# mryab/learning-at-home

Measured on NVIDIA H100. Metric: DMoE training samples/sec (whole job, device-timed, max over ranks), higher is better.
Workload: dtype bf16

## Files before the change

### learning-at-home_b200/csrc/moe.cu

```cuda
#include <cfloat>

#include "sm90.cuh"

namespace lah {

constexpr int MAX_WORLD = 8;
constexpr int MAX_GRID_DIMS = 4;
constexpr int MAX_K = 8;
constexpr long long SPIN_TIMEOUT_CYCLES = 20000000000ll;

struct Peers {
    char* base[MAX_WORLD];
    int world;
    int me;
    unsigned long long* wait_ns;
    int* step_ctr;
    int spin_timeout_ms;
    char* mc_base;
};

__device__ __forceinline__ void multimem_st_release_u32(void* mc_addr, int v) {
    asm volatile("multimem.st.release.sys.global.u32 [%0], %1;" ::"l"(mc_addr), "r"(v) : "memory");
}
__device__ __forceinline__ void multimem_st_u32(void* mc_addr, int v) {
// ... 611 lines not shown
}

__global__ void alive_from_heartbeats_kernel(const long long* hb, unsigned char* alive, int E, long long now_ms, long long max_age_ms) {
    const int e = blockIdx.x * blockDim.x + threadIdx.x;
    if (e < E) alive[e] = (hb[e] > 0 && now_ms - hb[e] <= max_age_ms) ? 1 : 0;
}

__global__ void step_begin_kernel(int* step_ctr, int epoch_delta, long long token_delta) {
    step_ctr[0] += epoch_delta;
    *reinterpret_cast<long long*>(step_ctr + 2) += token_delta;
}

struct CombineArgs {
    long long src_off;
    const int* idx;
    const int* pair_row;
    const float* w;
    bf16* out;
    int B, k, H, E_loc;
    long long flags_off;
    int slot, epoch, do_signal, do_wait;
    int* status;
    const int* route_owner;
};

template <int VEC_PER_LANE, bool ADD>
__global__ void __launch_bounds__(256) combine_rows_kernel(Peers peers, CombineArgs a, const bf16* __restrict__ addend) {
    const int warp = threadIdx.x >> 5, lane = threadIdx.x & 31;
    if (a.do_signal || a.do_wait) a.epoch = epoch_of(peers, a.epoch);
    if (a.do_signal && blockIdx.x == 0 && threadIdx.x < 32) {
        signal_all_ranks(peers, a.flags_off, a.slot, a.epoch, threadIdx.x);
    }
    if (a.do_wait) {
        if (threadIdx.x < peers.world) {
            const int* f = reinterpret_cast<const int*>(peers.base[peers.me] + a.flags_off) + a.slot * MAX_WORLD + threadIdx.x;
            const unsigned long long t0 = globaltimer_ns();
            spin_until_ge(f, a.epoch, a.status, peers.spin_timeout_ms, threadIdx.x);
            if (blockIdx.x == 0) account_wait(peers, t0, peers.world);
        }
        __syncthreads();
    }
    const int b = blockIdx.x * 8 + warp;
    if (b >= a.B) return;
    float acc[VEC_PER_LANE * 8];
    if constexpr (ADD) {
        const int4* ap = reinterpret_cast<const int4*>(addend + static_cast<long long>(b) * a.H);
#pragma unroll
        for (int v = 0; v < VEC_PER_LANE; ++v) {
            const int4 q = __ldg(ap + v * 32 + lane);
            const uint32_t u[4] = {(uint32_t)q.x, (uint32_t)q.y, (uint32_t)q.z, (uint32_t)q.w};
#pragma unroll
            for (int t = 0; t < 4; ++t) {
// ... 517 lines not shown
    if (!g_peers_set) return -10;
    ScatterArgs a;
    a.src = (const bf16*)src; a.scale = scale; a.idx = idx; a.pos = pos; a.dst_row = dst_row; a.pair_row = pair_row;
    a.dst_off = dst_off; a.flags_off = flags_off; a.slot = slot; a.epoch = epoch; a.num_pairs = num_pairs; a.k = k;
    a.H = H; a.E_loc = E_loc; a.max_rows = max_rows; a.group_off = group_off; a.group_rows = group_rows;
    a.pair_blocks = (num_pairs + 7) / 8; a.align = align; a.done_counter = done_counter; a.status = status;
    a.route_owner = route_owner; a.num_groups = num_groups > 0 ? num_groups : E_loc;
    const int pad_blocks = a.num_groups < 64 ? a.num_groups : 64;
    const int grid = a.pair_blocks + pad_blocks;
    if (H == 256) scatter_rows_kernel<1><<<grid, 256, 0, st>>>(g_peers, a);
    else if (H == 512) scatter_rows_kernel<2><<<grid, 256, 0, st>>>(g_peers, a);
    else if (H == 1024) scatter_rows_kernel<4><<<grid, 256, 0, st>>>(g_peers, a);
    else return -2;
    return -(int)cudaGetLastError();
}

int lah_signal_wait(long long flags_off, int slot, int epoch, int do_signal, int do_wait, int* status,
                    cudaStream_t st) {
    if (!g_peers_set) return -10;
    signal_wait_kernel<<<1, 32, 0, st>>>(g_peers, flags_off, slot, epoch, do_signal, do_wait, status);
    return -(int)cudaGetLastError();
}

int lah_combine_rows(long long src_off, const int* idx, const int* pair_row, const float* w, void* out, int B, int k,
                     int H, int E_loc, long long flags_off, int slot, int epoch, int do_signal, int do_wait, int* status,
                     const int* route_owner, const void* addend, cudaStream_t st) {
    if (!g_peers_set) return -10;
    if (B <= 0) return 0;
    CombineArgs a;
    a.src_off = src_off; a.idx = idx; a.pair_row = pair_row; a.w = w; a.out = (bf16*)out; a.B = B; a.k = k; a.H = H;
    a.E_loc = E_loc; a.flags_off = flags_off; a.slot = slot; a.epoch = epoch; a.do_signal = do_signal; a.do_wait = do_wait;
    a.status = status; a.route_owner = route_owner;
    const int grid = (B + 7) / 8;
    const bf16* add = (const bf16*)addend;
    if (add && (reinterpret_cast<uintptr_t>(add) % 16)) return -3;
#define LAH_COMBINE(V)                                                                   \
    if (add) combine_rows_kernel<V, true><<<grid, 256, 0, st>>>(g_peers, a, add);        \
    else combine_rows_kernel<V, false><<<grid, 256, 0, st>>>(g_peers, a, nullptr);
    if (H == 256) { LAH_COMBINE(1) }
    else if (H == 512) { LAH_COMBINE(2) }
    else if (H == 1024) { LAH_COMBINE(4) }
    else return -2;
#undef LAH_COMBINE
    return -(int)cudaGetLastError();
}

int lah_gate_bwd(long long yo_off, const void* grad, const int* idx, const int* pair_row, const float* w,
                 float* dlogits, int B, int k, int H, int E_loc, const int* grid_sizes, int ndim, const int* route_owner,
                 cudaStream_t st) {
    if (!g_peers_set) return -10;
    if (B <= 0) return 0;
    GridSpec gs;
// ... 104 lines not shown
```

### learning-at-home_b200/csrc/small_m.cu

```cuda
#include "sm90.cuh"
#include <climits>

namespace lah {
namespace smallm {

constexpr int BM = 128;
constexpr int BK = 64;
constexpr int MMA_K = 16;
constexpr int BN_MAX = 128;
constexpr int NUM_THREADS = 288;

namespace sab {

constexpr int STAGES = 6;
constexpr int A_BYTES = BM * BK * 2;
constexpr int B_BYTES = BN_MAX * BK * 2;
constexpr int STAGE_BYTES = A_BYTES + B_BYTES;
constexpr int BAR_OFFSET = STAGES * STAGE_BYTES;
constexpr int QD = 4;
constexpr int MAX_G = 1023;
constexpr int CUM_OFFSET = BAR_OFFSET + (2 * STAGES + 2 * QD) * 8 + QD * 4 + 16;
constexpr int SMEM_TOTAL = CUM_OFFSET + (MAX_G + 1) * 4 + 1024;
static_assert(SMEM_TOTAL <= 232448, "shared memory budget");

struct Params {
    int G, M_out, K;
    const int* group_off;
// ... 136 lines not shown
    const int num_kb = p.K / BK;

    if (warp == 8) {
        if (lane != 0) return;
        if (p.wait_flags) {
            const int epoch = p.wait_epoch + (p.epoch_base ? *p.epoch_base : 0);
            const unsigned long long t_wait = globaltimer_ns();
            for (int sidx = 0; sidx < p.wait_count; ++sidx)
                spin_flag_ft(p.wait_flags + sidx, epoch, p.status, sidx, p.epoch_base ? p.epoch_base[1] : 0);
            if (blockIdx.x == 0) atomicAdd(reinterpret_cast<unsigned long long*>(p.status + 2), globaltimer_ns() - t_wait);
            fence_proxy_async_global();
        }
        int stage = 0, qi = 0;
        uint32_t phase = 0, qphase = 0;
        while (true) {
            const int tile = atomicAdd(p.tile_counter, 1);
            mbar_wait(&q_empty[qi], qphase ^ 1);
            q_tile[qi] = tile;
            mbar_arrive(&q_full[qi]);
            if (++qi == QD) {
                qi = 0;
                qphase ^= 1;
            }
            if (tile >= total) break;
            const int gc = tile / m_slices, ms = tile - gc * m_slices;
            const int g = find_group(cum, p.G, gc);
            const int n0 = (gc - cum[g]) * BN_MAX;
            const int rows = __ldg(p.group_rows + g);
            const int off = __ldg(p.group_off + g);
            const int box = box_rows_of(min(rows - n0, BN_MAX));
            const CUtensorMap* tmB = box == 16 ? &tmB16 : (box == 32 ? &tmB32 : (box == 64 ? &tmB64 : &tmB128));
            for (int kb = 0; kb < num_kb; ++kb) {
                mbar_wait(&empty_bar[stage], phase ^ 1);
                uint8_t* sa = smem + stage * STAGE_BYTES;
                uint8_t* sb = sa + A_BYTES;
                const int k = kb * BK;
                mbar_arrive_expect_tx(&full_bar[stage], A_BYTES + box * 128);
                if (!A_MN) {
                    tma_load_3d(sa, &tmA, &full_bar[stage], k, ms * BM, g);
                } else {
#pragma unroll
                    for (int i = 0; i < BM / 64; ++i)
                        tma_load_3d(sa + i * (BK * 128), &tmA, &full_bar[stage], ms * BM + i * 64, k, g);
                }
                tma_load_2d(sb, tmB, &full_bar[stage], k, off + n0);
                if (++stage == STAGES) {
                    stage = 0;
// ... 53 lines not shown
static_assert(ST_STAGES <= CHUNKS, "the producer issues a tile's first ST_STAGES chunks before its remaining k-blocks");
static_assert(OP_STAGE_BYTES % 1024 == 0 && SUB_BYTES % 1024 == 0, "128-B swizzle atoms need 1 KB alignment");
static_assert(SMEM_TOTAL <= 232448, "shared memory budget");

struct Params {
    int G, N, K;
    const int* group_off;
    const int* group_rows;
    const int* skip;
    const int* step;
    float* p;
    float* m;
    float* v;
    float* vmax;
    bf16* p_bf16;
    float lr, beta1, beta2, eps;
    int amsgrad;
    float wd;
    int* tile_counter;
    const int* poison;
};
static_assert(sizeof(Params) == 128 && sizeof(Params) % alignof(CUtensorMap) == 0, "Params layout");

constexpr int WD_NONE = 0, WD_L2 = 1, WD_DECOUPLED = 2;

struct Tile {
    int g, mt, nt;
};

template <bool SPLIT>
struct StateMaps {
    CUtensorMap a[SPLIT ? 5 : 4];
};
constexpr int PLANE_COLS = 64;
constexpr int PLANE_BYTES = ARR_BYTES / 2;
static_assert(PLANE_BYTES == (BN_MAX / PLANE_COLS) * SUB_BYTES, "a plane box has the rows and bytes of an fp32 box");

template <bool SPLIT>
__device__ __forceinline__ void state_chunk_tma(const StateMaps<SPLIT>& tm, int n_arr, uint8_t* ss, uint64_t* bar, int col0,
                                                int srow, int c) {
    if constexpr (SPLIT) {
        for (int a = 0; a < 2; ++a)
#pragma unroll
            for (int q = 0; q < BN_MAX / PLANE_COLS; ++q) {
                uint8_t* s = ss + a * PLANE_BYTES + q * SUB_BYTES;
                if (bar) tma_load_3d(s, &tm.a[a], bar, col0 + q * PLANE_COLS, BAND_ROWS * c, srow / 16);
                else tma_store_3d(&tm.a[a], s, col0 + q * PLANE_COLS, BAND_ROWS * c, srow / 16);
            }
    }
    for (int a = SPLIT ? 1 : 0; a < n_arr; ++a)
#pragma unroll
        for (int q = 0; q < BN_MAX / SUB_COLS; ++q) {
            uint8_t* s = ss + a * ARR_BYTES + q * SUB_BYTES;
            const CUtensorMap* m = &tm.a[SPLIT ? a + 1 : a];
            if (bar) tma_load_3d(s, m, bar, col0 + q * SUB_COLS, BAND_ROWS * c, srow / 16);
            else tma_store_3d(m, s, col0 + q * SUB_COLS, BAND_ROWS * c, srow / 16);
        }
}

template <int WD, bool DEV_LR, bool SPLIT>
__global__ void __launch_bounds__(NUM_THREADS, 1)
wgrad_adam_kernel(const Params p, const __grid_constant__ CUtensorMap tmDY, const __grid_constant__ CUtensorMap tmX,
                  const __grid_constant__ StateMaps<SPLIT> tmS, const float* __restrict__ lr_dev) {
    extern __shared__ uint8_t smem_raw[];
    uint8_t* smem = reinterpret_cast<uint8_t*>((reinterpret_cast<uintptr_t>(smem_raw) + 1023) & ~uintptr_t(1023));
    uint8_t* st_smem = smem + ST_OFFSET;
    uint64_t* op_full = reinterpret_cast<uint64_t*>(smem + BAR_OFFSET);
    uint64_t* op_empty = op_full + OP_STAGES;
    uint64_t* st_full = op_empty + OP_STAGES;
    uint64_t* st_empty = st_full + ST_STAGES;
    uint64_t* q_full = st_empty + ST_STAGES;
    uint64_t* q_empty = q_full + QD;
    volatile int* q_tile = reinterpret_cast<volatile int*>(q_empty + QD);

    const int warp = threadIdx.x >> 5;
    const int lane = threadIdx.x & 31;
    if (p.poison && (*p.poison & 1)) return;
    const int n_arr = p.amsgrad ? 4 : 3;

    if (warp == 8 && lane == 0) {
        tma_prefetch_desc(&tmDY);
        tma_prefetch_desc(&tmX);
        for (int a = 0; a < n_arr + (SPLIT ? 1 : 0); ++a) tma_prefetch_desc(&tmS.a[a]);
        for (int i = 0; i < OP_STAGES; ++i) {
            mbar_init(&op_full[i], 1);
            mbar_init(&op_empty[i], 8);
        }
        for (int i = 0; i < ST_STAGES; ++i) {
            mbar_init(&st_full[i], 1);
            mbar_init(&st_empty[i], 1);
        }
        for (int i = 0; i < QD; ++i) {
            mbar_init(&q_full[i], 1);
            mbar_init(&q_empty[i], 8);
        }
        fence_mbar_init();
    }
    __syncthreads();

    const int n_tiles = p.K / BN_MAX;
    const int tiles_per_group = (p.N / BM) * n_tiles;
    const int total = p.G * tiles_per_group;
    auto decode = [&](int tile) {
        Tile t;
        t.g = tile / tiles_per_group;
        const int r = tile - t.g * tiles_per_group;
        t.mt = r / n_tiles;
        t.nt = r - t.mt * n_tiles;
        return t;
    };

    if (warp == 8) {
        if (lane != 0) return;
        uint32_t phase = 0, qphase = 0, sphase = 0;
        int qi = 0, stage = 0, sstage = 0;
        while (true) {
            int tile;
            while (true) {
                tile = atomicAdd(p.tile_counter, 1);
                if (tile >= total) break;
                const int g = tile / tiles_per_group;
                if (__ldg(p.group_rows + g) > 0 && !(p.skip && __ldg(p.skip + 2 * g) >= 0)) break;
                atomicMax(p.tile_counter, (g + 1) * tiles_per_group);
            }
            mbar_wait(&q_empty[qi], qphase ^ 1);
            q_tile[qi] = tile;
            mbar_arrive(&q_full[qi]);
            if (++qi == QD) {
                qi = 0;
                qphase ^= 1;
            }
            if (tile >= total) break;
            const Tile t = decode(tile);
            const int off = __ldg(p.group_off + t.g), rows = __ldg(p.group_rows + t.g);
            const int srow = t.g * p.N + t.mt * BM;
            auto load_chunk = [&](int c) {
                mbar_wait(&st_empty[sstage], sphase ^ 1);
                mbar_arrive_expect_tx(&st_full[sstage], n_arr * ARR_BYTES);
                state_chunk_tma(tmS, n_arr, st_smem + sstage * ST_STAGE_BYTES, &st_full[sstage], t.nt * BN_MAX, srow, c);
                if (++sstage == ST_STAGES) {
                    sstage = 0;
                    sphase ^= 1;
                }
// ... 164 lines not shown
                    acc[4 * j] = acc[4 * j + 2];
                    acc[4 * j + 1] = acc[4 * j + 3];
                }
            }
        }
    }
    if (threadIdx.x == 0) tma_store_wait<0>();
}

}
}
}

using namespace lah;
using namespace lah::smallm;

extern "C" const int* lah_get_epoch_base();

static int* tile_counter() {
    static int* ctr = nullptr;
    if (!ctr) {
        if (cudaMalloc(&ctr, 256) != cudaSuccess) return nullptr;
        cudaMemset(ctr, 0, 256);
    }
    return ctr;
}
static const int* g_poison = nullptr;

extern "C" {

int lah_set_poison_word(const int* status) {
    g_poison = status;
    return 0;
}
const int* lah_get_poison_word() { return g_poison; }

int lah_swapab_linear(const void* x, long long ldx, int x_rows, const void* W, int G, int M_out, int K, int a_mn,
                      void* out, long long ldo, const int* group_off, const int* group_rows, const float* bias,
                      const void* residual, long long ldr, const int* wait_flags, int wait_count, int wait_epoch,
                      int* status, int max_ctas, cudaStream_t st) {
    if ((K % BK) || (M_out % BM) || (ldx % 8) || G > sab::MAX_G) return -2;
    CUtensorMap tmA, tmB[4];
    if (!a_mn) {
        uint64_t dims[3] = {(uint64_t)K, (uint64_t)M_out, (uint64_t)G};
        uint64_t str[2] = {(uint64_t)K * 2, (uint64_t)M_out * K * 2};
        uint32_t box[3] = {BK, BM, 1};
        int r = make_tmap(&tmA, CU_TENSOR_MAP_DATA_TYPE_BFLOAT16, 3, W, dims, str, box);
        if (r) return r;
    } else {
        uint64_t dims[3] = {(uint64_t)M_out, (uint64_t)K, (uint64_t)G};
        uint64_t str[2] = {(uint64_t)M_out * 2, (uint64_t)M_out * K * 2};
        uint32_t box[3] = {64, BK, 1};
        int r = make_tmap(&tmA, CU_TENSOR_MAP_DATA_TYPE_BFLOAT16, 3, W, dims, str, box);
        if (r) return r;
    }
    const uint32_t boxes[4] = {16, 32, 64, 128};
    for (int i = 0; i < 4; ++i) {
        uint64_t dims[2] = {(uint64_t)K, (uint64_t)x_rows};
        uint64_t str[1] = {(uint64_t)ldx * 2};
        uint32_t box[2] = {BK, boxes[i]};
        int r = make_tmap(&tmB[i], CU_TENSOR_MAP_DATA_TYPE_BFLOAT16, 2, x, dims, str, box);
        if (r) return r;
    }
    sab::Params p;
    p.G = G; p.M_out = M_out; p.K = K; p.group_off = group_off; p.group_rows = group_rows; p.out = (bf16*)out; p.ldo = ldo;
    p.bias = bias; p.residual = (const bf16*)residual; p.ldr = ldr; p.wait_flags = wait_flags; p.wait_count = wait_count;
    p.wait_epoch = wait_epoch; p.epoch_base = lah_get_epoch_base(); p.status = status;
    p.tile_counter = tile_counter();
    if (!p.tile_counter) return -3;
    const long long total = 1ll * (M_out / BM) * (G + x_rows / BN_MAX);
    if (total <= 0 || G <= 0) return 0;
    if (cudaMemsetAsync(p.tile_counter, 0, sizeof(int), st) != cudaSuccess) return -4;
    const int ctas = persistent_grid(total, max_ctas);
    if (!a_mn) {
        if (int e = set_max_dynamic_smem<sab::swapab_kernel<false>>(sab::SMEM_TOTAL)) return e;
        sab::swapab_kernel<false><<<ctas, NUM_THREADS, sab::SMEM_TOTAL, st>>>(p, tmA, tmB[0], tmB[1], tmB[2], tmB[3]);
    } else {
        if (int e = set_max_dynamic_smem<sab::swapab_kernel<true>>(sab::SMEM_TOTAL)) return e;
        sab::swapab_kernel<true><<<ctas, NUM_THREADS, sab::SMEM_TOTAL, st>>>(p, tmA, tmB[0], tmB[1], tmB[2], tmB[3]);
    }
    return -(int)cudaGetLastError();
}

}

template <int WD, bool DEV_LR, bool SPLIT>
static int launch_wgrad_adam(const wa::Params& a, const CUtensorMap& tmDY, const CUtensorMap& tmX,
                             const wa::StateMaps<SPLIT>& tmS, const float* lr_dev, int ctas, cudaStream_t st) {
    if (int e = set_max_dynamic_smem<wa::wgrad_adam_kernel<WD, DEV_LR, SPLIT>>(wa::SMEM_TOTAL)) return e;
    wa::wgrad_adam_kernel<WD, DEV_LR, SPLIT><<<ctas, NUM_THREADS, wa::SMEM_TOTAL, st>>>(a, tmDY, tmX, tmS, lr_dev);
    return -(int)cudaGetLastError();
}

template <bool SPLIT>
static int wgrad_adam(const void* dy, long long lddy, const void* x, long long ldx, int total_rows, int G, int N, int K,
                      const int* group_off, const int* group_rows, const int* skip, const int* step, void* p, void* lo,
                      float* m, float* v, float* vmax, void* p_bf16, float lr, const float* lr_dev, float beta1, float beta2,
                      float eps, int amsgrad, float weight_decay, float decay, int decoupled, int max_ctas, cudaStream_t st) {
    if ((N % BM) || (K % BN_MAX) || (lddy % 8) || (ldx % 8) || 1ll * G * N > INT_MAX) return -2;
    if (decoupled && weight_decay != 0.f) return -2;
    if (amsgrad && !vmax) return -2;
    CUtensorMap tmDY, tmX;
    wa::StateMaps<SPLIT> tmS;
    {
        void* arrs[5] = {p, m, v, amsgrad ? vmax : (float*)m, nullptr};
        if (SPLIT) {
            arrs[1] = lo; arrs[2] = m; arrs[3] = v; arrs[4] = amsgrad ? vmax : m;
        }
        uint64_t dims[3] = {(uint64_t)K, 16, (uint64_t)G * N / 16};
        uint64_t str[2] = {(uint64_t)K * 4, (uint64_t)K * 64};
        uint32_t box[3] = {wa::SUB_COLS, wa::BAND_ROWS, BM / 16};
        for (int a = 0; a < (SPLIT ? 5 : 4); ++a) {
            int r;
            if (SPLIT && a < 2) {
                uint64_t pstr[2] = {(uint64_t)K * 2, (uint64_t)K * 32};
                uint32_t pbox[3] = {wa::PLANE_COLS, wa::BAND_ROWS, BM / 16};
                r = make_tmap(&tmS.a[a], CU_TENSOR_MAP_DATA_TYPE_BFLOAT16, 3, arrs[a], dims, pstr, pbox);
            } else {
                r = make_tmap(&tmS.a[a], CU_TENSOR_MAP_DATA_TYPE_FLOAT32, 3, arrs[a], dims, str, box);
            }
            if (r) return r;
// ... 2 lines not shown
    {
        uint64_t dims[2] = {(uint64_t)N, (uint64_t)total_rows};
        uint64_t str[1] = {(uint64_t)lddy * 2};
        uint32_t box[2] = {64, wa::WBK};
        int r = make_tmap(&tmDY, CU_TENSOR_MAP_DATA_TYPE_BFLOAT16, 2, dy, dims, str, box);
        if (r) return r;
    }
    {
        uint64_t dims[2] = {(uint64_t)K, (uint64_t)total_rows};
        uint64_t str[1] = {(uint64_t)ldx * 2};
        uint32_t box[2] = {64, wa::WBK};
        int r = make_tmap(&tmX, CU_TENSOR_MAP_DATA_TYPE_BFLOAT16, 2, x, dims, str, box);
        if (r) return r;
    }
    wa::Params a;
    a.G = G; a.N = N; a.K = K; a.group_off = group_off; a.group_rows = group_rows; a.skip = skip; a.step = step;
    a.p = SPLIT ? nullptr : (float*)p; a.m = m; a.v = v; a.vmax = vmax; a.p_bf16 = (bf16*)p_bf16; a.lr = lr; a.beta1 = beta1; a.beta2 = beta2; a.eps = eps; a.amsgrad = amsgrad;
    a.wd = decoupled ? decay : weight_decay;
    a.tile_counter = tile_counter() ? tile_counter() + 16 : nullptr;
    a.poison = g_poison;
    if (!a.tile_counter) return -3;
    const long long total = 1ll * G * (N / BM) * (K / BN_MAX);
    if (total <= 0) return 0;
    if (cudaMemsetAsync(a.tile_counter, 0, sizeof(int), st) != cudaSuccess) return -4;
    const int ctas = persistent_grid(total, max_ctas);
    if (lr_dev) {
        if (decoupled) return launch_wgrad_adam<wa::WD_DECOUPLED, true, SPLIT>(a, tmDY, tmX, tmS, lr_dev, ctas, st);
        if (weight_decay != 0.f) return launch_wgrad_adam<wa::WD_L2, true, SPLIT>(a, tmDY, tmX, tmS, lr_dev, ctas, st);
        return launch_wgrad_adam<wa::WD_NONE, true, SPLIT>(a, tmDY, tmX, tmS, lr_dev, ctas, st);
    }
    if (decoupled) return launch_wgrad_adam<wa::WD_DECOUPLED, false, SPLIT>(a, tmDY, tmX, tmS, nullptr, ctas, st);
    if (weight_decay != 0.f) return launch_wgrad_adam<wa::WD_L2, false, SPLIT>(a, tmDY, tmX, tmS, nullptr, ctas, st);
    return launch_wgrad_adam<wa::WD_NONE, false, SPLIT>(a, tmDY, tmX, tmS, nullptr, ctas, st);
}

extern "C" {

int lah_wgrad_adam(const void* dy, long long lddy, const void* x, long long ldx, int total_rows, int G, int N, int K,
                   const int* group_off, const int* group_rows, const int* skip, const int* step, float* p, float* m,
                   float* v, float* vmax, void* p_bf16, float lr, const float* lr_dev, float beta1, float beta2, float eps,
                   int amsgrad, float weight_decay, float decay, int decoupled, int max_ctas, cudaStream_t st) {
    return wgrad_adam<false>(dy, lddy, x, ldx, total_rows, G, N, K, group_off, group_rows, skip, step, p, nullptr, m, v,
                             vmax, p_bf16, lr, lr_dev, beta1, beta2, eps, amsgrad, weight_decay, decay, decoupled, max_ctas,
                             st);
}

int lah_wgrad_adam_split(const void* dy, long long lddy, const void* x, long long ldx, int total_rows, int G, int N, int K,
                         const int* group_off, const int* group_rows, const int* skip, const int* step, void* hi, void* lo,
                         float* m, float* v, float* vmax, float lr, const float* lr_dev, float beta1, float beta2, float eps,
                         int amsgrad, float weight_decay, float decay, int decoupled, int max_ctas, cudaStream_t st) {
    if (!hi || !lo) return -2;
    return wgrad_adam<true>(dy, lddy, x, ldx, total_rows, G, N, K, group_off, group_rows, skip, step, hi, lo, m, v, vmax,
                            nullptr, lr, lr_dev, beta1, beta2, eps, amsgrad, weight_decay, decay, decoupled, max_ctas, st);
}

}
```

### learning-at-home_b200/ops/kernels.py

```python
import ctypes
import math

import torch
import torch.nn.functional as F

from . import native
from .native import c_void_p, c_int, c_ll, c_float, ptr, stream_ptr

c_ull = ctypes.c_ulonglong
_configured = False

SLOT_COUNTS, SLOT_DISPATCH, SLOT_OUTPUT, SLOT_GRAD, SLOT_DINPUT, SLOT_TRAINER, SLOT_BARRIER, SLOT_SHADOW = range(8)
NUM_SLOTS = 8
MAX_WORLD = 8
STATUS_TIMEOUT, STATUS_OVERFLOW = 1, 2


def _lib():
    global _configured
    lib = native.cuda_lib()
    if _configured:
        return lib
    P, I, L, Fl = c_void_p, c_int, c_ll, c_float
    sigs = {
        "lah_ln_relu_fwd": [P, P, P, P, P, P, P, I, I, I, I, P],
        "lah_ln_relu_bwd": [P, P, P, P, P, P, P, P, P, P, P, P, I, I, I, I, P, P],
        "lah_grouped_colsum": [P, L, P, P, I, P, I, I, P],
        "lah_set_step_counters": [P],
        "lah_set_multicast": [c_ull],
        "lah_set_poison_word": [P],
        "lah_nvls_allreduce": [L, L, Fl, P],
        "lah_heartbeat": [L, I, I, L, P],
        "lah_alive_from_heartbeats": [P, P, I, L, L, P],
        "lah_set_spin_timeout_ms": [I],
        "lah_step_begin": [I, L, P],
        "lah_swapab_linear": [P, L, I, P, I, I, I, I, P, L, P, P, P, P, L, P, I, I, P, I, P],
        "lah_wgrad_adam": [P, L, P, L, I, I, I, I, P, P, P, P, P, P, P, P, P, Fl, P, Fl, Fl, Fl, I, Fl, Fl, I, I, P],
        "lah_wgrad_adam_split": [P, L, P, L, I, I, I, I, P, P, P, P, P, P, P, P, P, Fl, P, Fl, Fl, Fl, I, Fl, Fl, I, I, P],
        "lah_ln_relu_fwd_q": [P, P, P, P, P, P, P, I, I, I, P, P, P],
        "lah_set_peers": [P, I, I],
        "lah_set_wait_counter": [P],
        "lah_gate_topk": [P, I, P, I, I, P, Fl, c_ull, L, P, P, P, P, P, P],
        "lah_expert_bias_update": [P, I, I, P, Fl, P, P],
        "lah_layout_exchange": [L, L, I, I, I, I, I, I, I, P, P, P, P, P, P, P, I, Fl, I, P, P, P, P, P],
        "lah_scatter_rows": [P, P, P, P, P, P, L, L, I, I, I, I, I, I, I, I, P, P, P, P, P, I, P],
        "lah_pull_shadow": [P, I, I, L, L, I, P, I, P],
        "lah_zero_slots": [P, I, P, I, I, I, I, P],
        "lah_signal_wait": [L, I, I, I, I, P, P],
        "lah_combine_rows": [L, P, P, P, P, I, I, I, I, L, I, I, I, I, P, P, P, P],
        "lah_gate_bwd": [L, P, P, P, P, P, I, I, I, I, P, I, P, P],
        "lah_router_loss_fwd": [P, I, P, I, P, P, I, P, P, P, P, P, P, P],
        "lah_router_loss_bwd": [P, I, P, I, P, P, P, P, Fl, Fl, P, P],
        "lah_adam_step": [P, P, P, P, P, P, I, P, I, P, P, I, Fl, P, Fl, Fl, Fl, Fl, I, I, I, L, P, Fl, I, P, L, I, I, I, Fl,
                          I, P],
        "lah_bump_steps": [P, P, I, P],
        "lah_cast_bf16": [P, P, L, P],
        "lah_split_master": [P, P, P, P, L, I, P],
        "lah_attention_fwd": [P, P, P, L, I, I, I, c_ull, I, Fl, P, P],
        "lah_attention_bwd": [P, P, P, P, P, P, P, L, I, I, I, c_ull, I, Fl, P, P],
        "lah_attention_fwd_causal": [P, P, P, L, I, I, I, c_ull, I, Fl, P],
        "lah_attention_bwd_causal": [P, P, P, P, P, P, P, L, I, I, I, c_ull, I, Fl, P],
        "lah_pack_key_mask": [P, P, L, I, P],
        "lah_dropout_mask": [P, I, I, I, I, I, c_ull, I, P],
        "lah_dropout_ew": [I, P, P, P, L, I, c_ull, I, I, Fl, P],
        "lah_rms_norm_fwd": [P, P, P, P, I, I, Fl, P, I, P],
        "lah_rms_norm_bwd": [P, P, P, P, P, P, P, I, I, I, P, P, P],
        "lah_swiglu_fwd": [P, P, L, I, P],
        "lah_swiglu_bwd": [P, P, P, L, I, P],
        "lah_symm_alloc": [c_ull, ctypes.POINTER(c_void_p)],
        "lah_symm_free": [P],
        "lah_symm_get_handle": [P, ctypes.c_char_p],
        "lah_symm_open_handle": [ctypes.c_char_p, ctypes.POINTER(c_void_p)],
# ... 277 lines not shown
    native.count_launch()


def scatter_rows(src, scale, idx, pos, dst_row, pair_row, dst_off, flags_off, slot, epoch, k, E_loc, max_rows,
                 group_off, group_rows, done_counter, status, align=128, route_owner=None, num_groups=0):
    num_pairs = idx.numel()
    H = src.shape[1]
    assert src.is_contiguous() and src.dtype == torch.bfloat16
    native.check(_lib().lah_scatter_rows(ptr(src), ptr(scale), ptr(idx), ptr(pos), ptr(dst_row), ptr(pair_row), dst_off,
                                         flags_off, slot, epoch, num_pairs, k, H, E_loc, max_rows, align, ptr(group_off),
                                         ptr(group_rows), ptr(done_counter), ptr(status), ptr(route_owner),
                                         int(num_groups), stream_ptr()),
                 "lah_scatter_rows")
    native.count_launch()


def signal_wait(flags_off, slot, epoch, status, *, signal=True, wait=True):
    native.check(_lib().lah_signal_wait(flags_off, slot, epoch, int(signal), int(wait), ptr(status), stream_ptr()),
                 "lah_signal_wait")
    native.count_launch()


def combine_rows(src_off, idx, pair_row, w, out, k, E_loc, *, flags_off=0, slot=0, epoch=0, signal=False, wait=False,
                 status=None, route_owner=None, addend=None):
    B, H = out.shape
    if addend is not None:
        _bf16_rows(addend, "combine_rows addend", (B, H))
        if addend.data_ptr() % 16:
            raise ValueError("combine_rows: the addend must be 16-byte aligned")
    native.check(_lib().lah_combine_rows(src_off, ptr(idx), ptr(pair_row), ptr(w), ptr(out), B, k, H, E_loc, flags_off,
                                         slot, epoch, int(signal), int(wait), ptr(status), ptr(route_owner),
                                         ptr(addend), stream_ptr()),
                 "lah_combine_rows")
    native.count_launch()
    return out


def combine_rows_ref(src, idx, pair_row, w=None, addend=None):
    present = ((idx >= 0) & (pair_row >= 0)).double()
    if w is not None:
        present = present * w.double()
    terms = src.double()[pair_row.clamp(min=0).long()] * present.unsqueeze(-1)
    total = terms.sum(1)
    if addend is not None:
        total = total + addend.double()
    return total.to(torch.bfloat16)


def gate_bwd(yo_off, grad, idx, pair_row, w, dlogits, k, E_loc, grid_size, route_owner=None):
    B, H = grad.shape
    assert grad.is_contiguous() and grad.dtype == torch.bfloat16 and dlogits.dtype == torch.float32
    native.check(_lib().lah_gate_bwd(yo_off, ptr(grad), ptr(idx), ptr(pair_row), ptr(w), ptr(dlogits), B, k, H, E_loc,
                                     ctypes.cast(_grid_array(grid_size), c_void_p), len(grid_size), ptr(route_owner),
                                     stream_ptr()),
                 "lah_gate_bwd")
# ... 391 lines not shown
                                          wait_epoch, ptr(wait_status), int(max_ctas), stream_ptr()),
                 "lah_swapab_linear")
    native.count_launch()
    return out


def swapab_linear_ref(x, w, group_off, group_rows, *, bias=None, residual=None, w_is_kn=False):
    off, rows = group_off.tolist(), group_rows.tolist()
    M_out = w.shape[2] if w_is_kn else w.shape[1]
    out = torch.zeros(x.shape[0], M_out, dtype=torch.float32, device=x.device)
    for g, (o, r) in enumerate(zip(off, rows)):
        if r <= 0:
            continue
        wg = w[g].float()
        y = x[o:o + r].float() @ (wg if w_is_kn else wg.t())
        if bias is not None:
            y = y + bias.view(w.shape[0], M_out)[g]
        if residual is not None:
            y = y + residual[o:o + r].float()
        out[o:o + r] = y
    return out


def wgrad_adam(dy, x, group_off, group_rows, *, p, m, v, vmax, p_bf16, step, skip=None, lr=1e-3, betas=(0.9, 0.999),
               eps=1e-8, amsgrad=True, weight_decay=0.0, decoupled=False, max_ctas=0, lr_dev=None, p_lo=None):
    G, N, Kd = (p if p_lo is None else p_lo).shape
    assert dy.shape[1] == N and x.shape[1] == Kd and dy.shape[0] == x.shape[0]
    assert dy.dtype == torch.bfloat16 and x.dtype == torch.bfloat16
    if p_lo is None:
        assert p.is_contiguous() and p.dtype == torch.float32
    else:
        assert p is None and p_lo.dtype == torch.int16 and p_bf16.dtype == torch.bfloat16
        assert p_lo.is_contiguous() and p_bf16.is_contiguous() and p_bf16.shape[1:] == p_lo.shape[1:]
    if amsgrad and vmax is None:
        raise ValueError("wgrad_adam: amsgrad needs a vmax tensor (vmax=None only with amsgrad=False)")
    if lr_dev is not None:
        _check_lr_dev(lr_dev)
    l2, decay = weight_decay_args(lr, weight_decay, decoupled)
    common = (ptr(dy), dy.stride(0), ptr(x), x.stride(0), dy.shape[0], G, N, Kd, ptr(group_off), ptr(group_rows),
              ptr(skip), ptr(step))
    tail = (lr, ptr(lr_dev), betas[0], betas[1], eps, int(amsgrad), l2, decay, int(bool(decoupled and weight_decay)),
            int(max_ctas), stream_ptr())
    if p_lo is None:
        native.check(_lib().lah_wgrad_adam(*common, ptr(p), ptr(m), ptr(v), ptr(vmax), ptr(p_bf16), *tail),
                     "lah_wgrad_adam")
    else:
        native.check(_lib().lah_wgrad_adam_split(*common, ptr(p_bf16), ptr(p_lo), ptr(m), ptr(v), ptr(vmax), *tail),
                     "lah_wgrad_adam_split")
    native.count_launch()


def bump_steps(step, group_rows):
    native.check(_lib().lah_bump_steps(ptr(step), ptr(group_rows), step.numel(), stream_ptr()), "lah_bump_steps")
    native.count_launch()


def cast_bf16(src, dst):
    assert src.dtype == torch.float32 and dst.dtype == torch.bfloat16 and src.numel() == dst.numel()
    native.check(_lib().lah_cast_bf16(ptr(src), ptr(dst), src.numel(), stream_ptr()), "lah_cast_bf16")
    native.count_launch()


def _check_split(p, hi, lo, v):
    n = p.numel()
    assert p.dtype == torch.float32 and hi.dtype == torch.bfloat16 and lo.dtype == torch.int16 and v.dtype == torch.float32
    assert hi.numel() == n and lo.numel() == n and v.numel() == n
    assert all(t.is_contiguous() and t.is_cuda for t in (p, hi, lo, v))


def split_encode(p, hi, lo, v):
    _check_split(p, hi, lo, v)
# ... 153 lines not shown
```

### learning-at-home_b200/parallel/engine.py

```python
import math
from dataclasses import dataclass, field
from typing import Dict, List, Optional, Sequence, Tuple

import torch
import torch.nn as nn
import torch.nn.functional as F

from ..models.layers import FFN_SEG_KEYS as REF_KEYS, FFN_SEG_NAMES as SEG_NAMES, FFN_SMALL_SEG_MASK as SMALL_SEG_MASK
from ..models.layers import EXPERT_LAYOUTS, GATED_LAYOUT, GatedFeedforwardBlock, gated_inner_dim
from ..ops import fp8, gemm, kernels as K, native
from ..ops.expert_blocks import (RowPlan, ffn_backward, ffn_forward, ffn_forward_fp8, swiglu_mlp_backward,
                                 swiglu_mlp_forward)

GATED_EPS = 1e-6
SHARED_SWAPAB_ROWS = 512
SHARED_PAD = 128


@dataclass
class DMoEConfig:
    hidden: int = 512
    grid_size: Tuple[int, ...] = (8, 8)
    k: int = 4
    num_layers: int = 4
# ... 181 lines not shown
        self.cnt_all, self.cnt_all_off = self.heap.alloc((K.MAX_WORLD, self.E), torch.int32)
        i32 = dict(dtype=torch.int32, device=self.device)
        self.counts = torch.zeros(self.E, **i32)
        self.done_counter = torch.zeros(1, **i32)
        self._status_buf = torch.zeros(4, **i32)
        self.status = self._status_buf[:1]
        self.wait_ns = self._status_buf[2:4].view(torch.int64)
        K.set_wait_counter(self.wait_ns)
        self.step_ctr = torch.zeros(4, **i32)
        K.set_step_counters(self.step_ctr)
        K.set_spin_timeout_ms(cfg.peer_timeout_ms)
        self.step_ctr[1] = int(cfg.peer_timeout_ms)
        self.dead_mask = 0
        import os as _os
        octas = int(_os.environ.get("LAH_OPTIMIZER_CTAS", cfg.optimizer_ctas))
        sms = torch.cuda.get_device_properties(self.device).multi_processor_count
        if octas < 0:
            octas = sms * (17 if self.world == 1 else 18) // 28
        self.opt_ctas = octas if (self.small and 0 < octas < sms - 8) else 0
        self.chain_ctas = sms - self.opt_ctas if self.opt_ctas else 0
        self.opt_stream = torch.cuda.Stream(self.device) if self.opt_ctas else None
        self._opt_pending = False
        self.defer_join = False
        K.set_poison_word(self.status)
        self._lr_written = K.lr_block_values(cfg.lr, cfg.weight_decay, cfg.decoupled_weight_decay)
        self.lr_dev = torch.tensor(self._lr_written, dtype=torch.float32, device=self.device)
        assert 2 * cfg.num_layers + 4 < self.EPOCH_STRIDE
        self.alive = torch.ones(self.E, dtype=torch.uint8, device=self.device)
        self.hb, self.hb_off = self.heap.alloc((self.E,), torch.int64)
        self.hb.zero_()
        self._hb_stream = None
        self.epoch = 0
        self.token_counter = 0
        from .profiler import StageTimer
        self.timer = StageTimer(enabled=False)
        self.gyd, self.gyd_off = self.heap.alloc((self.max_rows, H), torch.bfloat16)
        self.dxd, self.dxd_off = self.heap.alloc((self.max_rows, H), torch.bfloat16)
        if cfg.router_losses:
            blocks = -(-cfg.tokens_per_rank // K.ROUTER_WARPS)
            self.router_partials = torch.zeros(2 * blocks, dtype=torch.float32, device=self.device)
            self.router_ticket = torch.zeros(1, dtype=torch.int32, device=self.device)
        bf = dict(dtype=torch.bfloat16, device=self.device)
        for name, width in cfg.layout.buffers(H, cfg.inner)["scratch"].items():
            setattr(self, name, torch.empty(self.max_rows, width, **bf))
        if cfg.shared_inner_dim:
            Is, R = cfg.shared_inner_dim, -(-cfg.tokens_per_rank // SHARED_PAD) * SHARED_PAD
# ... 576 lines not shown
        K.scatter_rows(gy, w, idx, pos, None, pair_row, ws.gyd_off, c.flags_off, K.SLOT_GRAD, epoch, k, c.E_loc,
                       c.max_rows, ws.group_off, ws.group_rows, c.done_counter, c.status, align=c.align,
                       route_owner=ws.route_owner, num_groups=c.G_tot)
        if c.S:
            K.zero_slots(sh.g, sh.seg_sizes, c.G_tot, c.E_loc, c.S, sh.layout.small_mask)
        dxs = self._shared_expert_bwd(gy, x) if self.shared_inner else None
        if c.world > 1:
            K.signal_wait(c.flags_off, K.SLOT_GRAD, epoch, c.status, signal=False, wait=True)
        c.timer.mark("bwd_gate+dispatch_grad")
        plan, go, gr = self._expert_plan(), ws.group_off, sh.grads
        if c.small:
            opt, E = c.adam_kwargs(), self.E_loc
            main, side = torch.cuda.current_stream(c.device), c.opt_stream

            def wgrad(name, dy, xin):
                kw = dict(p=None, p_lo=sh.lo_views[name][:E], p_bf16=sh.bf16[name][:E]) if sh.split else \
                    dict(p=sh.raw_views[name][:E], p_bf16=sh.bf16[name])
                kw.update(m=sh.m_views[name][:E], v=sh.v_raw_views[name][:E],
                          vmax=sh.vmax_views[name][:E] if cfg.amsgrad else None, step=sh.step, **opt)
                if side is None:
                    K.wgrad_adam(dy, xin, go, ws.group_rows, **kw)
                    return
                side.wait_stream(main)
                with torch.cuda.stream(side):
                    K.wgrad_adam(dy, xin, go, ws.group_rows, max_ctas=c.opt_ctas, **kw)
                c._opt_pending = True

            K.bump_steps(sh.step, ws.step_rows)
        else:
            def wgrad(name, dy, xin):
                gemm.grouped_wgrad(dy, xin, go, c.G_tot, out=gr[name], accumulate=cfg.accumulate)

        if cfg.expert == "swiglu":
            swiglu_mlp_backward(plan, sh.bf16["w13"], sh.bf16["w2"], ws.n, ws.h, ws.a, ws.gyd, c.da, ws.dh13, c.dn, wgrad)
            K.rms_norm_bwd(c.dn, ws.xd, ws.rstd, sh.raw_views["g"], dx=c.dxd, dgamma=gr["g"], dres=ws.gyd,
                           tile_rows=plan.tile_rows, tile_group=plan.tile_group)
        else:
            ffn_backward(plan, sh.bf16, sh.raw_views, gr, ws.xd, (ws.h1, ws.a1, ws.h2, ws.a2),
                         (ws.mean1, ws.rstd1, ws.mean2, ws.rstd2), ws.gyd, c.da, ws.dh2, ws.dh1, c.dxd, wgrad)
        if c.small:
            small = sh.layout.small_mask
            K.adam_step(sh.p_raw, sh.g, sh.m, sh.v_raw, sh.vmax, sh.p_bf16, sh.seg_sizes, sh.slots, step=sh.step,
                        group_rows=ws.step_rows, zero_mask=small, G_active=self.E_loc, seg_mask=small, **opt)
            sh.w8_dirty = True
            c.timer.mark("expert_ffn_bwd(dgrad+ln+fused wgrad/AMSGrad)")
        else:
            c.timer.mark("expert_ffn_bwd(wgrad+dgrad+ln)")
            if c.S:
                K.signal_wait(c.flags_off, K.SLOT_SHADOW, epoch, c.status, signal=True, wait=True)
            self.apply_expert_gradients()
            c.timer.mark("expert_adam")
        dx = torch.empty(B, cfg.hidden, dtype=torch.bfloat16, device=gy.device)
        K.combine_rows(c.dxd_off, idx, pair_row, None, dx, k, c.E_loc, flags_off=c.flags_off, slot=K.SLOT_DINPUT,
                       epoch=epoch, signal=c.world > 1, wait=c.world > 1, status=c.status, route_owner=ws.route_owner,
                       addend=dxs)
        c.timer.mark("bwd_combine")
        return dx, dlogits

    def apply_expert_gradients(self):
        sh, cfg, ws, c = self.shard, self.cfg, self.ws, self.ctx
        rows, zero_mask = ws.step_rows, sh.layout.small_mask
        if cfg.accumulate:
            sh.pending_rows += ws.step_rows
            sh.pending_steps += (sh.pending_rows > 0).to(torch.int32)
            thr_rows, thr_steps = cfg.update_thresholds()
            due = (sh.pending_rows > 0) & ((sh.pending_rows >= thr_rows) | (sh.pending_steps >= thr_steps))
            sh.fire.copy_(due.to(torch.int32))
            sh.pending_rows.mul_(1 - sh.fire)
            sh.pending_steps.mul_(1 - sh.fire)
            rows, zero_mask = sh.fire, (1 << len(sh.layout.names)) - 1
        K.bump_steps(sh.step, rows)
        K.adam_step(sh.p_raw, sh.g, sh.m, sh.v_raw, sh.vmax, sh.p_bf16, sh.seg_sizes, sh.slots, step=sh.step,
                    group_rows=rows, **c.adam_kwargs(), zero_mask=zero_mask, G_active=self.E_loc, world=c.world,
                    peer_bases=c.heap.peer_bases if c.S else None, shadow_of=ws.owned_shadow if c.S else None,
                    shadow_g_off=sh.g_off, me=c.rank)
        sh.w8_dirty = True

    def failure_rate_ref(self) -> float:
# ... 129 lines not shown
```

### learning-at-home_b200/parallel/trainer.py

```python
import math
from typing import Optional

import torch
import torch.nn as nn
import torch.nn.functional as F

from ..ops import kernels as K, native
from .engine import DMoEConfig, EngineContext, DMoEClassifier


class PendingLoss:

    def __init__(self, event=None, host=None, value=None):
        self._event, self._host, self._value = event, host, value

    def result(self) -> float:
        if self._value is None:
            self._event.synchronize()
            self._value = float(self._host[0])
        return self._value


class DMoETrainer:
    def __init__(self, cfg: DMoEConfig, group=None, device: Optional[torch.device] = None, profile_stages: bool = False,
# ... 165 lines not shown

    def _step_eager(self, x: torch.Tensor, y: torch.Tensor) -> torch.Tensor:
        self.model.train()
        timer = self.ctx.timer if self.cuda else None
        if self.cuda:
            self.ctx.refresh_lr()
            self.ctx.begin_step()
            self.ctx.defer_join = True
        if timer is not None:
            timer.start()
        m = max(1, int(self.cfg.trainer_microbatches))
        if m == 1:
            logits = self.model(x)
            loss = F.cross_entropy(logits.float(), y)
            if timer is not None:
                timer.mark("head+loss")
            loss.backward()
            if not self.cuda:
                for block in self.model.blocks:
                    block.apply_expert_gradients_ref()
        else:
            assert x.shape[0] % m == 0, "trainer_microbatches must divide the batch"
            total = None
            for xm, ym in zip(x.chunk(m), y.chunk(m)):
                loss_m = F.cross_entropy(self.model(xm).float(), ym) / m
                loss_m.backward()
                if not self.cuda:
                    for block in self.model.blocks:
                        block.apply_expert_gradients_ref()
                else:
                    self.ctx.join_optimizer_stream()
                total = loss_m.detach() if total is None else total + loss_m.detach()
            loss = total
        if timer is not None:
            timer.mark("trainer_bwd(stem+gates)")
        if self._stale_ring is not None:
            with torch.no_grad():
                oldest = self._stale_ring[0].clone()
                if self._stale_ring.shape[0] > 1:
                    self._stale_ring[:-1] = self._stale_ring[1:].clone()
                self._stale_ring[-1].copy_(self.flat_g)
                self.flat_g.copy_(oldest)
        self._trainer_optimizer_step()
        if self.cuda:
            self.ctx.join_optimizer_stream()
            self.ctx.defer_join = False
        if timer is not None:
            timer.mark("trainer_adam")
# ... 192 lines not shown
```

Baseline: 13690.

## Let side-stream wgrad-Adam grid expand once the last backward combine finishes

The side-stream fused wgrad+Adam kernel now launches at the full persistent grid size instead of being capped at opt_ctas. CTAs beyond base_ctas exit immediately unless a 'chain done' word, set by the final layer-0 backward combine kernel, matches the current epoch, so extra SMs join the optimizer work only after the main backward chain has finished. Tile counters are now reset in-kernel by the last CTA to exit, via an exit ticket, which removes the per-launch memset. The cost is added atomics and a cross-stream device-side handshake, and a risk of correctness problems if the counter reset or the epoch check races.

```diff
diff --git a/learning-at-home_b200/csrc/moe.cu b/learning-at-home_b200/csrc/moe.cu
--- a/learning-at-home_b200/csrc/moe.cu
+++ b/learning-at-home_b200/csrc/moe.cu
@@ -657,12 +657,14 @@
     int slot, epoch, do_signal, do_wait;
     int* status;
     const int* route_owner;
+    int* chain_done;
 };
 
 template <int VEC_PER_LANE, bool ADD>
 __global__ void __launch_bounds__(256) combine_rows_kernel(Peers peers, CombineArgs a, const bf16* __restrict__ addend) {
     const int warp = threadIdx.x >> 5, lane = threadIdx.x & 31;
     if (a.do_signal || a.do_wait) a.epoch = epoch_of(peers, a.epoch);
+    if (a.chain_done && blockIdx.x == 0 && threadIdx.x == 0) *a.chain_done = epoch_of(peers, 0);
     if (a.do_signal && blockIdx.x == 0 && threadIdx.x < 32) {
         signal_all_ranks(peers, a.flags_off, a.slot, a.epoch, threadIdx.x);
     }
@@ -1226,12 +1228,16 @@
     return -(int)cudaGetLastError();
 }
 
+int* lah_chain_done_word();
+
 int lah_combine_rows(long long src_off, const int* idx, const int* pair_row, const float* w, void* out, int B, int k,
                      int H, int E_loc, long long flags_off, int slot, int epoch, int do_signal, int do_wait, int* status,
-                     const int* route_owner, const void* addend, cudaStream_t st) {
+                     const int* route_owner, const void* addend, int chain_done, cudaStream_t st) {
     if (!g_peers_set) return -10;
     if (B <= 0) return 0;
     CombineArgs a;
+    a.chain_done = chain_done ? lah_chain_done_word() : nullptr;
+    if (chain_done && !a.chain_done) return -3;
     a.src_off = src_off; a.idx = idx; a.pair_row = pair_row; a.w = w; a.out = (bf16*)out; a.B = B; a.k = k; a.H = H;
     a.E_loc = E_loc; a.flags_off = flags_off; a.slot = slot; a.epoch = epoch; a.do_signal = do_signal; a.do_wait = do_wait;
     a.status = status; a.route_owner = route_owner;
diff --git a/learning-at-home_b200/csrc/small_m.cu b/learning-at-home_b200/csrc/small_m.cu
--- a/learning-at-home_b200/csrc/small_m.cu
+++ b/learning-at-home_b200/csrc/small_m.cu
@@ -3,6 +3,14 @@
 
 namespace lah {
 namespace smallm {
+
+__device__ __forceinline__ void take_exit_ticket(int* ctr) {
+    __threadfence();
+    if (atomicAdd(ctr + 1, 1) == static_cast<int>(gridDim.x) - 1) {
+        atomicExch(ctr, 0);
+        atomicExch(ctr + 1, 0);
+    }
+}
 
 constexpr int BM = 128;
 constexpr int BK = 64;
@@ -185,7 +193,10 @@
                 qi = 0;
                 qphase ^= 1;
             }
-            if (tile >= total) break;
+            if (tile >= total) {
+                take_exit_ticket(p.tile_counter);
+                break;
+            }
             const int gc = tile / m_slices, ms = tile - gc * m_slices;
             const int g = find_group(cum, p.G, gc);
             const int n0 = (gc - cum[g]) * BN_MAX;
@@ -285,6 +296,12 @@
 };
 static_assert(sizeof(Params) == 128 && sizeof(Params) % alignof(CUtensorMap) == 0, "Params layout");
 
+struct Join {
+    const int* done;
+    const int* step_base;
+    int base_ctas;
+};
+
 constexpr int WD_NONE = 0, WD_L2 = 1, WD_DECOUPLED = 2;
 
 struct Tile {
@@ -324,7 +341,7 @@
 template <int WD, bool DEV_LR, bool SPLIT>
 __global__ void __launch_bounds__(NUM_THREADS, 1)
 wgrad_adam_kernel(const Params p, const __grid_constant__ CUtensorMap tmDY, const __grid_constant__ CUtensorMap tmX,
-                  const __grid_constant__ StateMaps<SPLIT> tmS, const float* __restrict__ lr_dev) {
+                  const __grid_constant__ StateMaps<SPLIT> tmS, const float* __restrict__ lr_dev, const Join join) {
     extern __shared__ uint8_t smem_raw[];
     uint8_t* smem = reinterpret_cast<uint8_t*>((reinterpret_cast<uintptr_t>(smem_raw) + 1023) & ~uintptr_t(1023));
     uint8_t* st_smem = smem + ST_OFFSET;
@@ -338,7 +355,15 @@
 
     const int warp = threadIdx.x >> 5;
     const int lane = threadIdx.x & 31;
-    if (p.poison && (*p.poison & 1)) return;
+    int idle = 0;
+    if (threadIdx.x == 0) {
+        idle = p.poison && (*p.poison & 1);
+        if (!idle && join.base_ctas > 0 && static_cast<int>(blockIdx.x) >= join.base_ctas)
+            idle = *reinterpret_cast<volatile const int*>(join.done) !=
+                   (join.step_base ? *reinterpret_cast<volatile const int*>(join.step_base) : 0);
+        if (idle) take_exit_ticket(p.tile_counter);
+    }
+    if (__syncthreads_or(idle)) return;
     const int n_arr = p.amsgrad ? 4 : 3;
 
     if (warp == 8 && lane == 0) {
@@ -381,7 +406,10 @@
             int tile;
             while (true) {
                 tile = atomicAdd(p.tile_counter, 1);
-                if (tile >= total) break;
+                if (tile >= total) {
+                    take_exit_ticket(p.tile_counter);
+                    break;
+                }
                 const int g = tile / tiles_per_group;
                 if (__ldg(p.group_rows + g) > 0 && !(p.skip && __ldg(p.skip + 2 * g) >= 0)) break;
                 atomicMax(p.tile_counter, (g + 1) * tiles_per_group);
@@ -592,12 +620,25 @@
     if (!ctr) {
         if (cudaMalloc(&ctr, 256) != cudaSuccess) return nullptr;
         cudaMemset(ctr, 0, 256);
+        cudaMemset(ctr + 32, 0xff, sizeof(int));
     }
     return ctr;
 }
 static const int* g_poison = nullptr;
 
 extern "C" {
+
+int* lah_chain_done_word() { return tile_counter() ? tile_counter() + 32 : nullptr; }
+
+int lah_work_counters(int* dst, cudaStream_t st) {
+    const int* w = tile_counter();
+    if (!w) return -3;
+    for (int i = 0; i < 5; ++i) {
+        const int src = (i / 2) * 16 + i % 2;
+        if (cudaMemcpyAsync(dst + i, w + src, sizeof(int), cudaMemcpyDeviceToDevice, st) != cudaSuccess) return -4;
+    }
+    return 0;
+}
 
 int lah_set_poison_word(const int* status) {
     g_poison = status;
@@ -640,7 +681,6 @@
     if (!p.tile_counter) return -3;
     const long long total = 1ll * (M_out / BM) * (G + x_rows / BN_MAX);
     if (total <= 0 || G <= 0) return 0;
-    if (cudaMemsetAsync(p.tile_counter, 0, sizeof(int), st) != cudaSuccess) return -4;
     const int ctas = persistent_grid(total, max_ctas);
     if (!a_mn) {
         if (int e = set_max_dynamic_smem<sab::swapab_kernel<false>>(sab::SMEM_TOTAL)) return e;
@@ -656,9 +696,10 @@
 
 template <int WD, bool DEV_LR, bool SPLIT>
 static int launch_wgrad_adam(const wa::Params& a, const CUtensorMap& tmDY, const CUtensorMap& tmX,
-                             const wa::StateMaps<SPLIT>& tmS, const float* lr_dev, int ctas, cudaStream_t st) {
+                             const wa::StateMaps<SPLIT>& tmS, const float* lr_dev, const wa::Join& join, int ctas,
+                             cudaStream_t st) {
     if (int e = set_max_dynamic_smem<wa::wgrad_adam_kernel<WD, DEV_LR, SPLIT>>(wa::SMEM_TOTAL)) return e;
-    wa::wgrad_adam_kernel<WD, DEV_LR, SPLIT><<<ctas, NUM_THREADS, wa::SMEM_TOTAL, st>>>(a, tmDY, tmX, tmS, lr_dev);
+    wa::wgrad_adam_kernel<WD, DEV_LR, SPLIT><<<ctas, NUM_THREADS, wa::SMEM_TOTAL, st>>>(a, tmDY, tmX, tmS, lr_dev, join);
     return -(int)cudaGetLastError();
 }
 
@@ -666,7 +707,9 @@
 static int wgrad_adam(const void* dy, long long lddy, const void* x, long long ldx, int total_rows, int G, int N, int K,
                       const int* group_off, const int* group_rows, const int* skip, const int* step, void* p, void* lo,
                       float* m, float* v, float* vmax, void* p_bf16, float lr, const float* lr_dev, float beta1, float beta2,
-                      float eps, int amsgrad, float weight_decay, float decay, int decoupled, int max_ctas, cudaStream_t st) {
+                      float eps, int amsgrad, float weight_decay, float decay, int decoupled, int max_ctas, int base_ctas,
+                      cudaStream_t st) {
+    if (base_ctas < 0) return -2;
     if ((N % BM) || (K % BN_MAX) || (lddy % 8) || (ldx % 8) || 1ll * G * N > INT_MAX) return -2;
     if (decoupled && weight_decay != 0.f) return -2;
     if (amsgrad && !vmax) return -2;
@@ -715,16 +758,16 @@
     if (!a.tile_counter) return -3;
     const long long total = 1ll * G * (N / BM) * (K / BN_MAX);
     if (total <= 0) return 0;
-    if (cudaMemsetAsync(a.tile_counter, 0, sizeof(int), st) != cudaSuccess) return -4;
+    const wa::Join join{lah_chain_done_word(), lah_get_epoch_base(), base_ctas};
     const int ctas = persistent_grid(total, max_ctas);
     if (lr_dev) {
-        if (decoupled) return launch_wgrad_adam<wa::WD_DECOUPLED, true, SPLIT>(a, tmDY, tmX, tmS, lr_dev, ctas, st);
-        if (weight_decay != 0.f) return launch_wgrad_adam<wa::WD_L2, true, SPLIT>(a, tmDY, tmX, tmS, lr_dev, ctas, st);
-        return launch_wgrad_adam<wa::WD_NONE, true, SPLIT>(a, tmDY, tmX, tmS, lr_dev, ctas, st);
-    }
-    if (decoupled) return launch_wgrad_adam<wa::WD_DECOUPLED, false, SPLIT>(a, tmDY, tmX, tmS, nullptr, ctas, st);
-    if (weight_decay != 0.f) return launch_wgrad_adam<wa::WD_L2, false, SPLIT>(a, tmDY, tmX, tmS, nullptr, ctas, st);
-    return launch_wgrad_adam<wa::WD_NONE, false, SPLIT>(a, tmDY, tmX, tmS, nullptr, ctas, st);
+        if (decoupled) return launch_wgrad_adam<wa::WD_DECOUPLED, true, SPLIT>(a, tmDY, tmX, tmS, lr_dev, join, ctas, st);
+        if (weight_decay != 0.f) return launch_wgrad_adam<wa::WD_L2, true, SPLIT>(a, tmDY, tmX, tmS, lr_dev, join, ctas, st);
+        return launch_wgrad_adam<wa::WD_NONE, true, SPLIT>(a, tmDY, tmX, tmS, lr_dev, join, ctas, st);
+    }
+    if (decoupled) return launch_wgrad_adam<wa::WD_DECOUPLED, false, SPLIT>(a, tmDY, tmX, tmS, nullptr, join, ctas, st);
+    if (weight_decay != 0.f) return launch_wgrad_adam<wa::WD_L2, false, SPLIT>(a, tmDY, tmX, tmS, nullptr, join, ctas, st);
+    return launch_wgrad_adam<wa::WD_NONE, false, SPLIT>(a, tmDY, tmX, tmS, nullptr, join, ctas, st);
 }
 
 extern "C" {
@@ -735,16 +778,18 @@
                    int amsgrad, float weight_decay, float decay, int decoupled, int max_ctas, cudaStream_t st) {
     return wgrad_adam<false>(dy, lddy, x, ldx, total_rows, G, N, K, group_off, group_rows, skip, step, p, nullptr, m, v,
                              vmax, p_bf16, lr, lr_dev, beta1, beta2, eps, amsgrad, weight_decay, decay, decoupled, max_ctas,
-                             st);
+                             0, st);
 }
 
 int lah_wgrad_adam_split(const void* dy, long long lddy, const void* x, long long ldx, int total_rows, int G, int N, int K,
                          const int* group_off, const int* group_rows, const int* skip, const int* step, void* hi, void* lo,
                          float* m, float* v, float* vmax, float lr, const float* lr_dev, float beta1, float beta2, float eps,
-                         int amsgrad, float weight_decay, float decay, int decoupled, int max_ctas, cudaStream_t st) {
+                         int amsgrad, float weight_decay, float decay, int decoupled, int max_ctas, int base_ctas,
+                         cudaStream_t st) {
     if (!hi || !lo) return -2;
     return wgrad_adam<true>(dy, lddy, x, ldx, total_rows, G, N, K, group_off, group_rows, skip, step, hi, lo, m, v, vmax,
-                            nullptr, lr, lr_dev, beta1, beta2, eps, amsgrad, weight_decay, decay, decoupled, max_ctas, st);
-}
-
-}
+                            nullptr, lr, lr_dev, beta1, beta2, eps, amsgrad, weight_decay, decay, decoupled, max_ctas,
+                            base_ctas, st);
+}
+
+}
diff --git a/learning-at-home_b200/ops/kernels.py b/learning-at-home_b200/ops/kernels.py
--- a/learning-at-home_b200/ops/kernels.py
+++ b/learning-at-home_b200/ops/kernels.py
@@ -36,7 +36,9 @@
         "lah_step_begin": [I, L, P],
         "lah_swapab_linear": [P, L, I, P, I, I, I, I, P, L, P, P, P, P, L, P, I, I, P, I, P],
         "lah_wgrad_adam": [P, L, P, L, I, I, I, I, P, P, P, P, P, P, P, P, P, Fl, P, Fl, Fl, Fl, I, Fl, Fl, I, I, P],
-        "lah_wgrad_adam_split": [P, L, P, L, I, I, I, I, P, P, P, P, P, P, P, P, P, Fl, P, Fl, Fl, Fl, I, Fl, Fl, I, I, P],
+        "lah_wgrad_adam_split": [P, L, P, L, I, I, I, I, P, P, P, P, P, P, P, P, P, Fl, P, Fl, Fl, Fl, I, Fl, Fl, I, I, I,
+                                 P],
+        "lah_work_counters": [P, P],
         "lah_ln_relu_fwd_q": [P, P, P, P, P, P, P, I, I, I, P, P, P],
         "lah_set_peers": [P, I, I],
         "lah_set_wait_counter": [P],
@@ -47,7 +49,7 @@
         "lah_pull_shadow": [P, I, I, L, L, I, P, I, P],
         "lah_zero_slots": [P, I, P, I, I, I, I, P],
         "lah_signal_wait": [L, I, I, I, I, P, P],
-        "lah_combine_rows": [L, P, P, P, P, I, I, I, I, L, I, I, I, I, P, P, P, P],
+        "lah_combine_rows": [L, P, P, P, P, I, I, I, I, L, I, I, I, I, P, P, P, I, P],
         "lah_gate_bwd": [L, P, P, P, P, P, I, I, I, I, P, I, P, P],
         "lah_router_loss_fwd": [P, I, P, I, P, P, I, P, P, P, P, P, P, P],
         "lah_router_loss_bwd": [P, I, P, I, P, P, P, P, Fl, Fl, P, P],
@@ -371,7 +373,7 @@
 
 
 def combine_rows(src_off, idx, pair_row, w, out, k, E_loc, *, flags_off=0, slot=0, epoch=0, signal=False, wait=False,
-                 status=None, route_owner=None, addend=None):
+                 status=None, route_owner=None, addend=None, chain_done=False):
     B, H = out.shape
     if addend is not None:
         _bf16_rows(addend, "combine_rows addend", (B, H))
@@ -379,7 +381,7 @@
             raise ValueError("combine_rows: the addend must be 16-byte aligned")
     native.check(_lib().lah_combine_rows(src_off, ptr(idx), ptr(pair_row), ptr(w), ptr(out), B, k, H, E_loc, flags_off,
                                          slot, epoch, int(signal), int(wait), ptr(status), ptr(route_owner),
-                                         ptr(addend), stream_ptr()),
+                                         ptr(addend), int(bool(chain_done)), stream_ptr()),
                  "lah_combine_rows")
     native.count_launch()
     return out
@@ -817,8 +819,14 @@
     return out
 
 
+def work_counters():
+    out = torch.empty(5, dtype=torch.int32, device="cuda")
+    native.check(_lib().lah_work_counters(ptr(out), stream_ptr()), "lah_work_counters")
+    return out
+
+
 def wgrad_adam(dy, x, group_off, group_rows, *, p, m, v, vmax, p_bf16, step, skip=None, lr=1e-3, betas=(0.9, 0.999),
-               eps=1e-8, amsgrad=True, weight_decay=0.0, decoupled=False, max_ctas=0, lr_dev=None, p_lo=None):
+               eps=1e-8, amsgrad=True, weight_decay=0.0, decoupled=False, max_ctas=0, base_ctas=0, lr_dev=None, p_lo=None):
     G, N, Kd = (p if p_lo is None else p_lo).shape
     assert dy.shape[1] == N and x.shape[1] == Kd and dy.shape[0] == x.shape[0]
     assert dy.dtype == torch.bfloat16 and x.dtype == torch.bfloat16
@@ -829,19 +837,21 @@
         assert p_lo.is_contiguous() and p_bf16.is_contiguous() and p_bf16.shape[1:] == p_lo.shape[1:]
     if amsgrad and vmax is None:
         raise ValueError("wgrad_adam: amsgrad needs a vmax tensor (vmax=None only with amsgrad=False)")
+    if base_ctas and p_lo is None:
+        raise ValueError("wgrad_adam: base_ctas needs a split master weight (p_lo)")
     if lr_dev is not None:
         _check_lr_dev(lr_dev)
     l2, decay = weight_decay_args(lr, weight_decay, decoupled)
     common = (ptr(dy), dy.stride(0), ptr(x), x.stride(0), dy.shape[0], G, N, Kd, ptr(group_off), ptr(group_rows),
               ptr(skip), ptr(step))
     tail = (lr, ptr(lr_dev), betas[0], betas[1], eps, int(amsgrad), l2, decay, int(bool(decoupled and weight_decay)),
-            int(max_ctas), stream_ptr())
+            int(max_ctas))
     if p_lo is None:
-        native.check(_lib().lah_wgrad_adam(*common, ptr(p), ptr(m), ptr(v), ptr(vmax), ptr(p_bf16), *tail),
+        native.check(_lib().lah_wgrad_adam(*common, ptr(p), ptr(m), ptr(v), ptr(vmax), ptr(p_bf16), *tail, stream_ptr()),
                      "lah_wgrad_adam")
     else:
-        native.check(_lib().lah_wgrad_adam_split(*common, ptr(p_bf16), ptr(p_lo), ptr(m), ptr(v), ptr(vmax), *tail),
-                     "lah_wgrad_adam_split")
+        native.check(_lib().lah_wgrad_adam_split(*common, ptr(p_bf16), ptr(p_lo), ptr(m), ptr(v), ptr(vmax), *tail,
+                                                 int(base_ctas), stream_ptr()), "lah_wgrad_adam_split")
     native.count_launch()
 
 
diff --git a/learning-at-home_b200/parallel/engine.py b/learning-at-home_b200/parallel/engine.py
--- a/learning-at-home_b200/parallel/engine.py
+++ b/learning-at-home_b200/parallel/engine.py
@@ -227,6 +227,7 @@
         self.opt_stream = torch.cuda.Stream(self.device) if self.opt_ctas else None
         self._opt_pending = False
         self.defer_join = False
+        self.last_backward = True
         K.set_poison_word(self.status)
         self._lr_written = K.lr_block_values(cfg.lr, cfg.weight_decay, cfg.decoupled_weight_decay)
         self.lr_dev = torch.tensor(self._lr_written, dtype=torch.float32, device=self.device)
@@ -849,8 +850,9 @@
                     K.wgrad_adam(dy, xin, go, ws.group_rows, **kw)
                     return
                 side.wait_stream(main)
+                grid = dict(base_ctas=c.opt_ctas) if sh.split else dict(max_ctas=c.opt_ctas)
                 with torch.cuda.stream(side):
-                    K.wgrad_adam(dy, xin, go, ws.group_rows, max_ctas=c.opt_ctas, **kw)
+                    K.wgrad_adam(dy, xin, go, ws.group_rows, **grid, **kw)
                 c._opt_pending = True
 
             K.bump_steps(sh.step, ws.step_rows)
@@ -878,9 +880,10 @@
             self.apply_expert_gradients()
             c.timer.mark("expert_adam")
         dx = torch.empty(B, cfg.hidden, dtype=torch.bfloat16, device=gy.device)
+        chain_done = c.opt_stream is not None and self.layer_index == 0 and c.last_backward
         K.combine_rows(c.dxd_off, idx, pair_row, None, dx, k, c.E_loc, flags_off=c.flags_off, slot=K.SLOT_DINPUT,
                        epoch=epoch, signal=c.world > 1, wait=c.world > 1, status=c.status, route_owner=ws.route_owner,
-                       addend=dxs)
+                       addend=dxs, chain_done=chain_done)
         c.timer.mark("bwd_combine")
         return dx, dlogits
 
diff --git a/learning-at-home_b200/parallel/trainer.py b/learning-at-home_b200/parallel/trainer.py
--- a/learning-at-home_b200/parallel/trainer.py
+++ b/learning-at-home_b200/parallel/trainer.py
@@ -211,8 +211,10 @@
         else:
             assert x.shape[0] % m == 0, "trainer_microbatches must divide the batch"
             total = None
-            for xm, ym in zip(x.chunk(m), y.chunk(m)):
+            for i, (xm, ym) in enumerate(zip(x.chunk(m), y.chunk(m))):
                 loss_m = F.cross_entropy(self.model(xm).float(), ym) / m
+                if self.cuda:
+                    self.ctx.last_backward = i == m - 1
                 loss_m.backward()
                 if not self.cuda:
                     for block in self.model.blocks:
```

Result: faster. 13920 (median of 6 runs) (+1.7%).
